# jedward225/MARL-HideAndSeek

Measured on AMD Instinct MI355X. Metric: world-steps/sec (agent-steps/sec derived) at 16K worlds, 1/2/4/8 GPU, higher is better.
Workload: dtype f32; 1 GPU; 16000 worlds/GPU x 2646 steps, 2 hiders + 2 seekers, sim_flags=0, rand_seed=0, random move actions in [-5,4] each step (scripts/benchmark.py args); worlds_per_gpu=16000, total_worlds=16000, agents_per_world=4

## Files before the change

__graft_entry__.py:

```python
import os
import sys

ROOT = os.path.dirname(os.path.abspath(__file__))
PKG = os.path.join(ROOT, "marl-hideandseek_amd")
for p in (PKG, os.path.join(ROOT, "oracle")):
    if p not in sys.path:
        sys.path.insert(0, p)


def build():
    import build as hs_build
    lib = hs_build.build_lib()
    hs_build.build_headless()
    hs_build.build_smallcap()
    import hs_ref
    hs_ref.build()
    import subprocess
    syms = ("hs_create", "hs_destroy", "hs_init", "hs_step", "hs_step_begin", "hs_step_end", "hs_step_async",
            "hs_get_tensor", "hs_train_interface", "hs_get_device_status", "hs_render", "hs_xla_init", "hs_xla_step",
            "hs_xla_save_checkpoints", "hs_xla_load_checkpoints", "hs_pack_policy_inputs", "hs_pack_policy_inputs_async")
    subprocess.check_call([sys.executable, "-c",
                           "import ctypes, sys; L = ctypes.CDLL(sys.argv[1]); [getattr(L, s) for s in sys.argv[2:]]", lib, *syms])
    subprocess.check_call([sys.executable, "-c", "import sys; sys.path.insert(0, sys.argv[1]); import gpu_hideseek", PKG])
    return lib


def smoke():
    import torch
    import lockstep
    assert torch.cuda.is_available(), "smoke() needs a GPU"
    p = lockstep.Pair(32, seed=7, render=(32, 32))
    p.drive(8, "bench", seed=0, every=8, walls=False,
            names=("self_data", "box_data", "lidar", "reward", "visible_boxes_mask"))
    p.sim.render()
    p.check_views(32, 32, "smoke")
    print("smoke OK: 8 steps x 32 worlds and their 128 agent views bit-exact vs oracle")


if __name__ == "__main__":
    if len(sys.argv) > 1 and sys.argv[1] == "smoke":
        smoke()
    else:
        print(build())
```

marl-hideandseek_amd/build.py:

```python
import os
import shutil
import subprocess
import sys

HERE = os.path.dirname(os.path.abspath(__file__))
CSRC = os.path.join(HERE, "csrc")
LIB = os.path.join(HERE, "lib", "libhideseek.so")

HIPCC_FLAGS = ["--offload-arch=gfx950", "-O3", "-fno-slp-vectorize", "-Wno-pass-failed", "-std=c++17", "-fPIC", "-shared", "-ffp-contract=off",
               "-fno-fast-math", "-Wno-unused-value"]


def sources():
    return sorted(os.path.join(CSRC, f) for f in os.listdir(CSRC) if f.endswith((".hip", ".h"))) + [
        os.path.join(os.path.dirname(HERE), "include", "hideseek.h")]


def up_to_date(lib=LIB):
    if not os.path.exists(lib):
        return False
    t = os.path.getmtime(lib)
    return all(os.path.getmtime(s) <= t for s in sources())


def build_lib(force=False, verbose=False, out=LIB, defines=()):
    if not force and up_to_date(out):
        return out
    hipcc = shutil.which("hipcc") or "/opt/rocm/bin/hipcc"
    if not os.path.exists(hipcc):
        raise RuntimeError("hipcc not found: cannot build libhideseek.so (there is no CPU fallback)")
    os.makedirs(os.path.dirname(out), exist_ok=True)
    cmd = [hipcc] + HIPCC_FLAGS + ["-D" + d for d in defines] + (
        ["-Rpass-analysis=kernel-resource-usage"] if verbose else []) + ["-o", out, os.path.join(CSRC, "hideseek.hip")]
    subprocess.check_call(cmd, cwd=CSRC)
    return out


SMALLCAP_LIB = os.path.join(HERE, "lib", "libhideseek_smallcap.so")


def build_smallcap(force=False):
    return build_lib(force=force, out=SMALLCAP_LIB, defines=("HS_MAX_DD_CAND=1", "HS_MAX_S_CAND=1"))


TIMING_LIB = os.path.join(HERE, "lib", "libhideseek_timing.so")


def build_timing(force=False):
    return build_lib(force=force, out=TIMING_LIB, defines=("HS_PHASE_TIMING",))


def build_headless():
    out = os.path.join(HERE, "lib", "headless")
    src = os.path.join(HERE, "tools", "headless.cpp")
    if os.path.exists(out) and os.path.getmtime(out) >= max(os.path.getmtime(src), os.path.getmtime(LIB)):
        return out
    subprocess.check_call(["g++", "-O2", "-std=c++17", "-I", os.path.join(os.path.dirname(HERE), "include"), src,
                           "-L", os.path.join(HERE, "lib"), "-lhideseek", "-Wl,-rpath,$ORIGIN", "-o", out])
    return out


if __name__ == "__main__":
    print(build_lib(force="--force" in sys.argv, verbose="-v" in sys.argv))
    print(build_headless())
    print(build_smallcap(force="--force" in sys.argv))
    if "--timing" in sys.argv:
        print(build_timing(force="--force" in sys.argv))
```

marl-hideandseek_amd/csrc/hs_dev.h:

```cpp
#pragma once
#include <hip/hip_runtime.h>
#include <stdint.h>

#define HSD __device__ __forceinline__

__device__ __forceinline__ int hs_lane() { int x = threadIdx.x; asm volatile("" : "+v"(x)); return x; }

namespace hs {

constexpr int kMaxBoxes = 9;
constexpr int kMaxRamps = 2;
constexpr int kMaxAgents = 6;
constexpr int kBoxSlot0 = 0;
constexpr int kRampSlot0 = 9;
constexpr int kAgentSlot0 = 11;
constexpr int kNumDSlots = 17;
constexpr int kMaxWalls = 36;
constexpr int kMaxPlanes = 3;
constexpr int kNumPrepSteps = 96;
constexpr int kEpisodeLen = 240;
constexpr int kNumSubsteps = 4;
constexpr float kSubstepH = (1.f / 30.f) / 4.f;
constexpr float kInvSubstepH = 120.f;
constexpr float kGravityZ = -9.8f;
constexpr float kMaxDepenVel = 3.f;
#ifndef HS_MAX_DD_CAND
#define HS_MAX_DD_CAND 16
#endif
#ifndef HS_MAX_S_CAND
#define HS_MAX_S_CAND 24
#endif
constexpr int kMaxDDCand = HS_MAX_DD_CAND;
constexpr int kGrabWords = 15;
constexpr int kMaxSCand = HS_MAX_S_CAND;
constexpr float kCosFovHalf = 0.382683426f;
constexpr float kPi = 3.14159265358979323846f;

enum : int { OBJ_SPHERE = 0, OBJ_PLANE = 1, OBJ_CUBE = 2, OBJ_WALL = 3, OBJ_HIDER = 4, OBJ_SEEKER = 5,
             OBJ_RAMP = 6, OBJ_BOX = 7, OBJ_NONE = -1 };
enum : int { OWNER_NONE = 0, OWNER_SEEKER = 1, OWNER_HIDER = 2, OWNER_UNOWNABLE = 3 };
enum : int { RESP_DYNAMIC = 0, RESP_KINEMATIC = 1, RESP_STATIC = 2 };
enum : int { AGENT_SEEKER = 0, AGENT_HIDER = 1 };
enum : uint32_t { FLAG_USE_FIXED_WORLD = 1, FLAG_IGNORE_EPISODE_LENGTH = 2, FLAG_RANDOM_FLIP_TEAMS = 4,
                  FLAG_ZERO_AGENT_VELOCITY = 8, FLAG_EXT_SKIP_OBSERVATIONS = 1u << 16, FLAG_EXT_RENDER = 1u << 17 };

HSD int meta_pack(int obj, int resp, int owner) { return (obj + 1) | (resp << 8) | (owner << 16); }
HSD int meta_obj(int m) { return (m & 0xff) - 1; }
HSD int meta_resp(int m) { return (m >> 8) & 0xff; }
HSD int meta_owner(int m) { return (m >> 16) & 0xff; }

struct V3 { float x, y, z; };
struct Q { float w, x, y, z; };

HSD V3 v3(float x, float y, float z) { return V3{x, y, z}; }
HSD V3 operator+(V3 a, V3 b) { return {a.x + b.x, a.y + b.y, a.z + b.z}; }
HSD V3 operator-(V3 a, V3 b) { return {a.x - b.x, a.y - b.y, a.z - b.z}; }
HSD V3 operator-(V3 a) { return {-a.x, -a.y, -a.z}; }
HSD V3 operator*(V3 a, float s) { return {a.x * s, a.y * s, a.z * s}; }
HSD V3 mulc(V3 a, V3 b) { return {a.x * b.x, a.y * b.y, a.z * b.z}; }
HSD float hs_fma(float a, float b, float c) { return __builtin_fmaf(a, b, c); }
HSD float dot(V3 a, V3 b) { return hs_fma(a.z, b.z, hs_fma(a.y, b.y, a.x * b.x)); }
HSD V3 cross(V3 a, V3 b) { return {hs_fma(a.y, b.z, -(a.z * b.y)), hs_fma(a.z, b.x, -(a.x * b.z)), hs_fma(a.x, b.y, -(a.y * b.x))}; }
HSD V3 madd(V3 a, V3 b, float s) { return {hs_fma(b.x, s, a.x), hs_fma(b.y, s, a.y), hs_fma(b.z, s, a.z)}; }
HSD V3 nmadd(V3 a, V3 b, float s) { return {hs_fma(-b.x, s, a.x), hs_fma(-b.y, s, a.y), hs_fma(-b.z, s, a.z)}; }
HSD float dot_add(V3 a, V3 b, float c) { return hs_fma(a.z, b.z, hs_fma(a.y, b.y, hs_fma(a.x, b.x, c))); }
HSD V3 cross_add(V3 a, V3 b, V3 c) {
    return {hs_fma(a.y, b.z, hs_fma(-a.z, b.y, c.x)), hs_fma(a.z, b.x, hs_fma(-a.x, b.z, c.y)), hs_fma(a.x, b.y, hs_fma(-a.y, b.x, c.z))};
}
HSD float len2(V3 a) { return dot(a, a); }
HSD float len(V3 a) { return sqrtf(dot(a, a)); }
HSD V3 normalize(V3 a) { float inv = 1.f / len(a); return a * inv; }
HSD V3 vsel(bool c, V3 a, V3 b) { return {c ? a.x : b.x, c ? a.y : b.y, c ? a.z : b.z}; }

HSD Q qmul(Q a, Q b) {
    return {hs_fma(-a.z, b.z, hs_fma(-a.y, b.y, hs_fma(-a.x, b.x, a.w * b.w))),
            hs_fma(-a.z, b.y, hs_fma(a.y, b.z, hs_fma(a.x, b.w, a.w * b.x))),
            hs_fma(a.z, b.x, hs_fma(a.y, b.w, hs_fma(-a.x, b.z, a.w * b.y))),
            hs_fma(a.z, b.w, hs_fma(-a.y, b.x, hs_fma(a.x, b.y, a.w * b.z)))};
}
HSD Q qinv(Q q) { return {q.w, -q.x, -q.y, -q.z}; }
HSD Q qnormalize(Q q) {
    float n2 = hs_fma(q.z, q.z, hs_fma(q.y, q.y, hs_fma(q.x, q.x, q.w * q.w)));
    float inv = 1.f / sqrtf(n2);
    return {q.w * inv, q.x * inv, q.y * inv, q.z * inv};
}
HSD V3 qrot(Q q, V3 v) {
    V3 p = {q.x, q.y, q.z};
    float s = q.w;
    float d2 = 2.f * dot(p, v);
    float s2 = 2.f * s;
    float k = hs_fma(s2, s, -1.f);
    V3 c = cross(p, v);
    return {hs_fma(s2, c.x, hs_fma(d2, p.x, k * v.x)), hs_fma(s2, c.y, hs_fma(d2, p.y, k * v.y)), hs_fma(s2, c.z, hs_fma(d2, p.z, k * v.z))};
}

HSD void hs_sincosf(float x, float *s_out, float *c_out) {
    const float two_over_pi = 0.63661977236758134308f;
    const float pio2_hi = 1.5707962512969970703125f;
    const float pio2_lo = 7.54978995489188216e-8f;
    float kf = x * two_over_pi;
    int k = (int)(kf + (kf >= 0.f ? 0.5f : -0.5f));
    float fk = (float)k;
    float r = (x - fk * pio2_hi) - fk * pio2_lo;
    float z = r * r;
    float sp = ((-1.9515295891e-4f * z + 8.3321608736e-3f) * z - 1.6666654611e-1f) * z * r + r;
    float cp = ((2.443315711809948e-5f * z - 1.388731625493765e-3f) * z + 4.166664568298827e-2f) * z * z
               - 0.5f * z + 1.f;
    int q = k & 3;
    float s = (q == 0) ? sp : (q == 1) ? cp : (q == 2) ? -sp : -cp;
    float c = (q == 0) ? cp : (q == 1) ? -sp : (q == 2) ? -cp : sp;
    *s_out = s; *c_out = c;
}
HSD float hs_atanf(float xin) {
    float sign = xin < 0.f ? -1.f : 1.f;
    float x = fabsf(xin);
    float y;
    const bool big = x > 2.414213562373095f, mid = x > 0.4142135623730950f;
    y = big ? 1.5707963267948966f : (mid ? 0.7853981633974483f : 0.f);
    if (mid) { const float num = big ? -1.f : x - 1.f, den = big ? x : x + 1.f; x = num / den; }
    float z = x * x;
    y = y + ((((8.05374449538e-2f * z - 1.38776856032e-1f) * z + 1.99777106478e-1f) * z - 3.33329491539e-1f) * z * x + x);
    return sign * y;
}
HSD float hs_atan2f(float y, float x) {
    if (x == 0.f) {
        if (y > 0.f) return 0.5f * kPi;
        if (y < 0.f) return -0.5f * kPi;
        return 0.f;
    }
    float a = hs_atanf(y / x);
    if (x < 0.f) { a = (y >= 0.f) ? a + kPi : a - kPi; }
    return a;
}
HSD float hs_asinf(float xin) {
    float sign = xin < 0.f ? -1.f : 1.f;
    float a = fabsf(xin);
    float z, x;
    bool flag = a > 0.5f;
    if (flag) { z = 0.5f * (1.f - a); x = sqrtf(z); }
    else { x = a; z = x * x; }
    float p = ((((4.2163199048e-2f * z + 2.4181311049e-2f) * z + 4.5470025998e-2f) * z + 7.4953002686e-2f) * z
               + 1.6666752422e-1f) * z * x + x;
    if (flag) { p = p + p; p = 1.5707963267948966f - p; }
    return sign * p;
}
HSD Q quat_angle_axis_z(float angle) {
    float s, c;
    hs_sincosf(angle * 0.5f, &s, &c);
    return {c, 0.f, 0.f, s};
}

struct M3 { V3 c0, c1, c2; };
HSD M3 m3_from_quat(Q q) {
    float y2 = q.y * q.y, z2 = q.z * q.z;
    float xy = q.x * q.y, xz = q.x * q.z, yz = q.y * q.z;
    M3 m;
    m.c0 = {hs_fma(-2.f, hs_fma(q.y, q.y, z2), 1.f), 2.f * hs_fma(q.w, q.z, xy), 2.f * hs_fma(-q.w, q.y, xz)};
    m.c1 = {2.f * hs_fma(-q.w, q.z, xy), hs_fma(-2.f, hs_fma(q.x, q.x, z2), 1.f), 2.f * hs_fma(q.w, q.x, yz)};
    m.c2 = {2.f * hs_fma(q.w, q.y, xz), 2.f * hs_fma(-q.w, q.x, yz), hs_fma(-2.f, hs_fma(q.x, q.x, y2), 1.f)};
    return m;
}

HSD V3 quat_to_euler(Q q) {
    float sinr = 2.f * (q.w * q.x + q.y * q.z);
    float cosr = 1.f - 2.f * (q.x * q.x + q.y * q.y);
    float roll = hs_atan2f(sinr, cosr);
    float sinp = 2.f * (q.w * q.y - q.z * q.x);
    float pitch = fabsf(sinp) >= 1.f ? copysignf(kPi / 2.f, sinp) : hs_asinf(sinp);
    float siny = 2.f * (q.w * q.z + q.x * q.y);
    float cosy = 1.f - 2.f * (q.y * q.y + q.z * q.z);
    float yaw = hs_atan2f(siny, cosy);
    return {roll, pitch, yaw};
}

struct RandKey { uint32_t a, b; };
HSD uint32_t rotl32(uint32_t x, int r) { return (x << r) | (x >> (32 - r)); }
HSD RandKey threefry2x32(RandKey key, uint32_t c0, uint32_t c1) {
    const uint32_t ks0 = key.a, ks1 = key.b, ks2 = 0x1BD11BDAu ^ key.a ^ key.b;
    uint32_t x0 = c0 + ks0, x1 = c1 + ks1;
#define HS_TF_R(r) { x0 += x1; x1 = rotl32(x1, r); x1 ^= x0; }
    HS_TF_R(13) HS_TF_R(15) HS_TF_R(26) HS_TF_R(6)
    x0 += ks1; x1 += ks2 + 1u;
    HS_TF_R(17) HS_TF_R(29) HS_TF_R(16) HS_TF_R(24)
    x0 += ks2; x1 += ks0 + 2u;
    HS_TF_R(13) HS_TF_R(15) HS_TF_R(26) HS_TF_R(6)
    x0 += ks0; x1 += ks1 + 3u;
    HS_TF_R(17) HS_TF_R(29) HS_TF_R(16) HS_TF_R(24)
// ... 43 lines not shown
```

marl-hideandseek_amd/csrc/hs_k_physics.h:

```cpp
#pragma once
#include "hs_state.h"
#include "hs_rays.h"
#include "hs_collide.h"
#include "hs_solver.h"
#include "hs_k_reset.h"

namespace hs {

constexpr int kPhysThreads = 64;
constexpr int kWorldLanes = kPhysThreads / kTile;
constexpr int kLdsWalls = 32;
static_assert(kMaxSCand <= 32 && kMaxDDCand <= 16, "accepted-manifold masks are one word per world");
constexpr int kAllDD = kNumDSlots * (kNumDSlots - 1) / 2;
constexpr int kAllSC = kNumDSlots * (kMaxWalls + kMaxPlanes - 1);
constexpr int kSpInfoWords = kNumDSlots + 1;

struct alignas(16) OctRes {
    static constexpr int kClip = kClipLanes;
    static constexpr int kClipWords = clip_words(kClip);
    static constexpr int kSatPairs = kClip < hs::kSatPairs ? kClip : hs::kSatPairs;
    static constexpr int kMaxItems = kTile * (kMaxDDCand + kMaxSCand);
    static constexpr int kSlots = kClip < 31 ? kClip : 31;
    static constexpr int kVelOffsetWords = 2 * 8 * 3 * 32;
    float pos[3][kNumDSlots][kTile];
// ... 36 lines not shown
};
static_assert(sizeof(OctRes) <= 20 * 1024, "8 waves of 8 worlds share the CU's 160 KiB of LDS");
static_assert(offsetof(OctRes, u.sat.items) >= offsetof(OctRes, u.det.wall), "items must not overlap the AABBs");
static_assert(sizeof(ManDD) / 4 * OctRes::kSlots <= OctRes::kVelOffsetWords, "manifold slots lie below the velocities");
static_assert(2 * 3 * kNumDSlots * 8 <= OctRes::kVelOffsetWords, "the hull AABBs lie below the velocities");

constexpr int kLocGlobal = 31;
HSD int pair_a(int p) { return p & 31; }
HSD int pair_b(int p) { return (p >> 5) & 63; }
HSD int pair_loc(int p) { return (p >> 11) & 31; }
HSD int pair_pack(int a, int b) { return a | (b << 5) | (kLocGlobal << 11); }
static_assert(kNumDSlots <= 32 && kMaxWalls + kMaxPlanes <= 64, "pair encoding");
static_assert(sizeof(ManDD) % 16 == 0 && sizeof(ManS) % 16 == 0, "manifold records move 16 bytes at a time");
constexpr int kManWords = sizeof(ManDD) / 4;
template <typename M> HSD void man_lds_load(const float *clip, int slot, M &m) {
    m = *reinterpret_cast<const M *>(clip + slot * kManWords);
}
template <typename M> HSD void man_lds_set_lam(float *clip, int slot, int j, float v) {
    static_assert(offsetof(M, lam) == sizeof(M) - 16, "lam is the record's tail");
    clip[slot * kManWords + (sizeof(M) / 4 - 4 + j)] = v;
}

template <int C> HSD V3 rld3(const float (&a)[C][kNumDSlots][kTile], int slot, int g) { return {a[0][slot][g], a[1][slot][g], a[2][slot][g]}; }
HSD Q rld4(const float (&a)[4][kNumDSlots][kTile], int slot, int g) { return {a[0][slot][g], a[1][slot][g], a[2][slot][g], a[3][slot][g]}; }
HSD void rst3(float (&a)[3][kNumDSlots][kTile], int slot, int g, V3 v) { a[0][slot][g] = v.x; a[1][slot][g] = v.y; a[2][slot][g] = v.z; }
HSD void rst4(float (&a)[4][kNumDSlots][kTile], int slot, int g, Q q) { a[0][slot][g] = q.w; a[1][slot][g] = q.x; a[2][slot][g] = q.y; a[3][slot][g] = q.z; }

HSD void rbody_load(const OctRes &R, int g, int slot, BodyS &b) {
    b.pos = rld3(R.pos, slot, g); b.rot = rld4(R.rot, slot, g);
    b.ppos = rld3(R.ppos, slot, g); b.prot = rld4(R.prot, slot, g);
    b.lin = rld3(R.u.vel.lin, slot, g); b.ang = rld3(R.u.vel.ang, slot, g);
    const int m = R.meta[slot][g];
    const bool dyn = m != 0 && meta_resp(m) == RESP_DYNAMIC;
    b.invM = dyn ? obj_inv_mass(meta_obj(m)) : 0.f;
    b.invI = dyn ? obj_inv_inertia(meta_obj(m)) : V3{0.f, 0.f, 0.f};
    body_refresh_inertia(b);
}
HSD void rbody_store_pose(OctRes &R, int g, int slot, const BodyS &b) { rst3(R.pos, slot, g, b.pos); rst4(R.rot, slot, g, b.rot); }
HSD void rbody_store_vel(OctRes &R, int g, int slot, const BodyS &b) { rst3(R.u.vel.lin, slot, g, b.lin); rst3(R.u.vel.ang, slot, g, b.ang); }
HSD void derive_velocity(BodyS &b) {
    const float h = kSubstepH;
    b.lin = (b.pos - b.ppos) * (1.f / h);
    Q dq = qmul(b.rot, qinv(b.prot));
    V3 wv = V3{dq.x, dq.y, dq.z} * (2.f / h);
    b.ang = dq.w >= 0.f ? wv : -wv;
}

HSD void wave_sync() { asm volatile("s_waitcnt lgkmcnt(0)" ::: "memory"); }
HSD void mem_sync() { asm volatile("s_waitcnt vmcnt(0) lgkmcnt(0)" ::: "memory"); }

template <int D> HSD int dpp_row_shr(int x) { return __builtin_amdgcn_update_dpp(0, x, 0x110 + D, 0xF, 0xF, true); }
HSD int scan8_incl(int x, int l) {
    int y;
    y = dpp_row_shr<1>(x); if (l >= 1) x += y;
    y = dpp_row_shr<2>(x); if (l >= 2) x += y;
    y = dpp_row_shr<4>(x); if (l >= 4) x += y;
    return x;
}
HSD int sum8_all(int x) {
    x += __builtin_amdgcn_update_dpp(0, x, 0xB1, 0xF, 0xF, false);
    x += __builtin_amdgcn_update_dpp(0, x, 0x4E, 0xF, 0xF, false);
    x += __builtin_amdgcn_update_dpp(0, x, 0x141, 0xF, 0xF, false);
    return x;
}
HSD int scan64_incl(int x) {
    x += dpp_row_shr<1>(x); x += dpp_row_shr<2>(x); x += dpp_row_shr<4>(x); x += dpp_row_shr<8>(x);
    x += __builtin_amdgcn_update_dpp(0, x, 0x142, 0xA, 0xF, false);
    x += __builtin_amdgcn_update_dpp(0, x, 0x143, 0xC, 0xF, false);
    return x;
}

struct ResGeom {
    const OctRes &R; const SimState &S; int g; int w;
    HSD int g_meta(int i) const { return R.meta[i][g]; }
    HSD V3 g_pos(int i) const { return rld3(R.pos, i, g); }
    HSD Q g_rot(int i) const { return rld4(R.rot, i, g); }
    HSD int g_num_walls() const { return R.numWalls[g]; }
    HSD float g_wall(int k, int c) const { return S.walls(c * kMaxWalls + k, w); }
    HSD int g_num_planes() const { return R.numPlanes[g]; }
    HSD float g_plane(int p, int c) const { return S.planes(c * kMaxPlanes + p, w); }
};

constexpr float kGroundOff = 0.f;
struct BodyReg {
    int np, vidx;
    float lam[4];
};

template <typename E, int ROWS>
HSD void copy_in(E *dst, const Col<E, ROWS> &col, int p0) {
    static_assert(sizeof(E) == 4, "16-byte pieces");
    const float4 *src = reinterpret_cast<const float4 *>(col.octet(p0 >> 3));
    float4 *d = reinterpret_cast<float4 *>(dst);
    for (int i = hs_lane(); i < ROWS * 2; i += 64) d[i] = src[(i / 2) * 2 + i % 2];
}
template <typename E, int ROWS>
HSD void copy_out(const Col<E, ROWS> &col, int p0, const E *src) {
    static_assert(sizeof(E) == 4, "16-byte pieces");
    float4 *dst = reinterpret_cast<float4 *>(col.octet(p0 >> 3));
    const float4 *s = reinterpret_cast<const float4 *>(src);
    for (int i = hs_lane(); i < ROWS * 2; i += 64) dst[(i / 2) * 2 + i % 2] = s[i];
}
HSD void copy_out_vel(const Col<float, 3 * kNumDSlots> &col, int p0, const float *src, const OctRes &R) {
    float *dst = col.octet(p0 >> 3);
    for (int i = hs_lane(); i < 3 * kNumDSlots * kTile; i += 64) {
        const int row = i / kTile, g = i % kTile, slot = row % kNumDSlots;
        const int m = R.meta[slot][g];
        if (m != 0 && meta_resp(m) == RESP_DYNAMIC) dst[row * kTile + g] = src[i];
    }
}

HSD void integrate_body(OctRes &R, BodyReg &b, int slot, int g, int meta, const float *aforce) {
    const int obj = meta_obj(meta);
    const bool dyn = meta_resp(meta) == RESP_DYNAMIC;
    V3 force = {0.f, 0.f, 0.f}; float torque = 0.f;
    if (dyn && slot >= kAgentSlot0) {
        const float *f = aforce + (slot - kAgentSlot0) * kTile + g;
        force = {f[0 * kMaxAgents * kTile], f[1 * kMaxAgents * kTile], f[2 * kMaxAgents * kTile]};
        torque = f[3 * kMaxAgents * kTile];
    }
    V3 pos = rld3(R.pos, slot, g); Q rot = rld4(R.rot, slot, g);
    rst3(R.ppos, slot, g, pos); rst4(R.prot, slot, g, rot);
    if (dyn) {
        V3 lin = rld3(R.u.vel.lin, slot, g), ang = rld3(R.u.vel.ang, slot, g);
        const float h = kSubstepH;
        const float invM = obj_inv_mass(obj);
        const V3 invI = obj_inv_inertia(obj);
        lin = madd(lin, madd(V3{0.f, 0.f, kGravityZ}, force, invM), h);
        pos = madd(pos, lin, h);
        Q qi = qinv(rot);
        V3 wloc = qrot(qi, ang), tl = qrot(qi, V3{0.f, 0.f, torque});
        const V3 I = obj_inertia(obj);
        V3 Iw = mulc(I, wloc);
        wloc = madd(wloc, mulc(invI, tl - cross(wloc, Iw)), h);
        ang = qrot(rot, wloc);
        rot = quat_add_rotation(rot, ang * h);
        rst3(R.pos, slot, g, pos); rst4(R.rot, slot, g, rot);
        rst3(R.u.vel.lin, slot, g, lin); rst3(R.u.vel.ang, slot, g, ang);
    }
    V3 lo, hi;
    const HullRef hb = hull_ref_body(obj, pos, rot);
    hull_aabb(hb, &lo, &hi);
    rst3(R.u.det.lo, slot, g, lo); rst3(R.u.det.hi, slot, g, hi);
    b.np = 0; b.vidx = 0;
#pragma unroll
    for (int j = 0; j < 4; ++j) b.lam[j] = 0.f;
    if (dyn && R.numPlanes[g] >= 1) {
        const V3 pn = {R.plane0[0][g], R.plane0[1][g], R.plane0[2][g]};
        b.np = ground_manifold(hb, pn, R.plane0[3][g], &b.vidx);
    }
}

struct ItemCounts { int nbox, nwedge; bool anySpill; };
template <int JB>
HSD ItemCounts phase_detect(const SimState &S, OctRes &R, int NS) {
    constexpr int G = kWorldLanes;
    const int L = hs_lane(), g = L / G, l = L % G;
    {
        constexpr int PR = kTile / 4;
        static_assert(kLdsWalls * PR <= 64, "one piece per lane per component");
        const float *src = S.walls.octet(S.wbeg >> 3);
        float4 v[4];
        const bool on = L < kLdsWalls * PR;
        const int row = L / PR, part = L % PR;
#pragma unroll
        for (int c = 0; c < 4; ++c) if (on) v[c] = *(const float4 *)(src + (c * kMaxWalls + row) * kTile + 4 * part);
#pragma unroll
        for (int c = 0; c < 4; ++c) if (on) *(float4 *)(&R.u.det.wall[c][row][4 * part]) = v[c];
    }
    if (l == 0) { R.scAcc[g] = 0u; R.ddAcc[g] = 0u; }
    wave_sync();
    const int nwl = R.numWalls[g], npl = R.numPlanes[g];
    int tot_items = 0;
    unsigned dd_mask[JB] = {}; unsigned long long s_mask[JB] = {};
    int bdd[JB] = {}, bsc[JB] = {}, add[JB] = {}, asc[JB] = {};
    bool have[JB], dynamic[JB]; V3 lo[JB], hi[JB];
#pragma unroll
    for (int jb = 0; jb < JB; ++jb) {
        const int slot = l + jb * G;
        const int meta = slot < NS ? R.meta[slot][g] : 0;
        have[jb] = meta != 0;
        dynamic[jb] = have[jb] && meta_resp(meta) == RESP_DYNAMIC;
        lo[jb] = {0.f, 0.f, 0.f}; hi[jb] = {0.f, 0.f, 0.f};
        if (have[jb]) { lo[jb] = rld3(R.u.det.lo, slot, g); hi[jb] = rld3(R.u.det.hi, slot, g); }
    }
#pragma unroll 4
    for (int j = 1; j < NS; ++j) {
        const int mj = R.meta[j][g];
        const bool dynj = meta_resp(mj) == RESP_DYNAMIC;
        const V3 loj = rld3(R.u.det.lo, j, g), hij = rld3(R.u.det.hi, j, g);
#pragma unroll
        for (int jb = 0; jb < JB; ++jb) {
            const bool hit = (mj != 0) & have[jb] & (l + jb * G < j) & (dynamic[jb] | dynj) &
                (lo[jb].x <= hij.x) & (loj.x <= hi[jb].x) & (lo[jb].y <= hij.y) & (loj.y <= hi[jb].y) &
                (lo[jb].z <= hij.z) & (loj.z <= hi[jb].z);
            dd_mask[jb] |= hit ? 1u << j : 0u;
        }
    }
    bool zin[JB];
#pragma unroll
    for (int jb = 0; jb < JB; ++jb) zin[jb] = dynamic[jb] & (lo[jb].z <= 2.5f) & (0.f <= hi[jb].z);
    auto wall_test = [&](int k, float cx, float cy, float hx, float hy) {
        const float wx0 = cx - hx, wx1 = cx + hx, wy0 = cy - hy, wy1 = cy + hy;
#pragma unroll
        for (int jb = 0; jb < JB; ++jb) {
            const bool hit = zin[jb] & (lo[jb].x <= wx1) & (wx0 <= hi[jb].x) & (lo[jb].y <= wy1) & (wy0 <= hi[jb].y);
            s_mask[jb] |= hit ? 1ull << k : 0ull;
        }
    };
    const int nwLds = nwl < kLdsWalls ? nwl : kLdsWalls;
#pragma unroll 4
    for (int k = 0; k < nwLds; ++k) wall_test(k, R.u.det.wall[0][k][g], R.u.det.wall[1][k][g], R.u.det.wall[2][k][g], R.u.det.wall[3][k][g]);
    for (int k = kLdsWalls; k < nwl; ++k) {
        const int w = S.wbeg + g;
        wall_test(k, S.walls(0 * kMaxWalls + k, w), S.walls(1 * kMaxWalls + k, w), S.walls(2 * kMaxWalls + k, w), S.walls(3 * kMaxWalls + k, w));
    }
    int tot_dd = 0, tot_sc = 0;
#pragma unroll
    for (int jb = 0; jb < JB; ++jb) {
        if (dynamic[jb]) for (int p = 1; p < npl; ++p) s_mask[jb] |= 1ull << (kMaxWalls + p);
        const int cdd = __popc(dd_mask[jb]), csc = __popcll(s_mask[jb]);
        const int in_dd = scan8_incl(cdd, l), in_sc = scan8_incl(csc, l);
        bdd[jb] = tot_dd + in_dd - cdd; bsc[jb] = tot_sc + in_sc - csc;
        tot_dd += sum8_all(cdd); tot_sc += sum8_all(csc);
        add[jb] = cdd ? max(0, min(cdd, kMaxDDCand - bdd[jb])) : 0;
        asc[jb] = csc ? max(0, min(csc, kMaxSCand - bsc[jb])) : 0;
        tot_items += add[jb] + asc[jb];
        if (add[jb] != cdd) atomicAdd(&S.status[0], cdd - add[jb]);
        if (asc[jb] != csc) atomicAdd(&S.status[1], csc - asc[jb]);
    }
    const bool spillDD = tot_dd > kMaxDDCand, spillSC = tot_sc > kMaxSCand;
    const bool anySpill = __ballot(spillDD || spillSC) != 0ull;
    unsigned short *const spPair = S.spPair + (size_t)(S.wbeg + g) * (kAllDD + kAllSC);
    int *const spInfo = S.spInfo + (size_t)(S.wbeg + g) * kSpInfoWords;
    int n_wedge = 0;
#pragma unroll
    for (int jb = 0; jb < JB; ++jb) {
        const int slot = l + jb * G;
        const bool ramp = slot >= kRampSlot0 && slot < kRampSlot0 + kMaxRamps;
        if (ramp) n_wedge += add[jb] + asc[jb];
        else { unsigned mm = dd_mask[jb]; for (int i = 0; mm && i < add[jb]; ++i) { const int j = __ffs(mm) - 1; mm &= mm - 1; n_wedge += (j >= kRampSlot0 && j < kRampSlot0 + kMaxRamps) ? 1 : 0; } }
    }
    const int n_box = tot_items - n_wedge;
    const int inc_box = scan64_incl(n_box), inc_wedge = scan64_incl(n_wedge);
    ItemCounts ic;
    ic.anySpill = anySpill;
    ic.nbox = __builtin_amdgcn_readlane(inc_box, 63); ic.nwedge = __builtin_amdgcn_readlane(inc_wedge, 63);
    const int wedge0 = (ic.nbox + 31) / 32 * 32;
    int ibox = inc_box - n_box, iwedge = wedge0 + inc_wedge - n_wedge;
    wave_sync();
#pragma unroll
    for (int jb = 0; jb < JB; ++jb) {
        const int slot = l + jb * G;
        const bool ramp = slot >= kRampSlot0 && slot < kRampSlot0 + kMaxRamps;
        unsigned mm = dd_mask[jb]; int i = 0;
        while (mm && i < add[jb]) {
            const int j = __ffs(mm) - 1; mm &= mm - 1;
            R.ddPair[bdd[jb] + i][g] = (unsigned short)pair_pack(slot, j);
            const unsigned short item = (unsigned short)((g << 6) | (bdd[jb] + i));
            if (ramp || (j >= kRampSlot0 && j < kRampSlot0 + kMaxRamps)) R.u.sat.items[iwedge++] = item; else R.u.sat.items[ibox++] = item;
            ++i;
        }
        while (mm) {
            const int j = __ffs(mm) - 1; mm &= mm - 1;
            spPair[bdd[jb] + i] = (unsigned short)pair_pack(slot, j);
            ++i;
        }
        unsigned long long sm = (s_mask[jb] >> kMaxWalls) | (s_mask[jb] << (64 - kMaxWalls) >> (64 - kMaxWalls) << kMaxPlanes); i = 0;
        while (sm && i < asc[jb]) {
            const int bit = __ffsll((long long)sm) - 1; sm &= sm - 1;
            const int k = bit < kMaxPlanes ? kMaxWalls + bit : bit - kMaxPlanes;
            R.scPair[bsc[jb] + i][g] = (unsigned short)pair_pack(slot, k);
            const unsigned short item = (unsigned short)((g << 6) | 32 | (bsc[jb] + i));
            if (ramp) R.u.sat.items[iwedge++] = item; else R.u.sat.items[ibox++] = item;
            ++i;
        }
        const int nspill = sm ? __popcll(sm) : 0;
        while (sm) {
            const int bit = __ffsll((long long)sm) - 1; sm &= sm - 1;
            const int k = bit < kMaxPlanes ? kMaxWalls + bit : bit - kMaxPlanes;
            spPair[kAllDD + bsc[jb] + i] = (unsigned short)pair_pack(slot, k);
            ++i;
        }
        if (spillSC && slot < kNumDSlots) spInfo[1 + slot] = nspill ? ((bsc[jb] + asc[jb]) | (nspill << 16)) : 0;
        if (slot < NS) R.scInfo[slot][g] = (unsigned short)(asc[jb] > 0 ? (bsc[jb] | (asc[jb] << 8)) : 0);
    }
    if (l == 0) {
        R.spill[g] = (unsigned char)((spillDD ? 1 : 0) | (spillSC ? 2 : 0));
        if (spillDD || spillSC) spInfo[0] = tot_dd | (tot_sc << 16);
        R.ndd[g] = (unsigned char)min(tot_dd, kMaxDDCand); R.nsc[g] = (unsigned char)min(tot_sc, kMaxSCand);
        if (R.wid[g] >= 0 && tot_dd + tot_sc > 0) S.loadAcc[R.wid[g]] += tot_dd + tot_sc;
    }
    wave_sync();
    return ic;
}

template <bool POS, int UNROLL, typename SetLam>
HSD void static_manifold(BodyS &me, const ManS &m, SetLam set_lam) {
    BodyS none;
    body_refresh_inertia(me);
    const V3 n = ld3(m.n);
    const int np = m.np;
    const float mu = POS ? m.muS : m.muD;
#pragma unroll UNROLL
    for (int j = 0; j < 4; ++j)
        if (j < np) {
            const float lamj = m.lam[j];
            if (POS) set_lam(j, lamj + solve_point_position<false>(me, none, n, ld3(m.rA[j]), V3{0.f, 0.f, 0.f}, m.offB[j], mu));
            else solve_point_velocity<false>(me, none, n, ld3(m.rA[j]), V3{0.f, 0.f, 0.f}, lamj, mu);
        }
}

#define HS_COLD __device__ __forceinline__
struct SpillCtx {
    const float *walls, *planes;
    ManDD *wsDD; ManS *wsSC; unsigned short *spPair; int *spInfo;
    int wbeg;
};
HSD SpillCtx spill_ctx(const SimState &S) { return {S.walls.p, S.planes.p, (ManDD *)S.wsDD, (ManS *)S.wsSC, S.spPair, S.spInfo, S.wbeg}; }

HS_COLD void spill_sat(SpillCtx c, OctRes *Rp) {
    OctRes &R = *Rp;
    const int lane = hs_lane() & 63;
    const bool hi = (lane & 1) != 0;
    const Col<float, 4 * kMaxWalls> walls = {const_cast<float *>(c.walls)};
    const Col<float, 4 * kMaxPlanes> planes = {const_cast<float *>(c.planes)};
#pragma unroll 1
    for (int g = 0; g < kTile; ++g) {
        const int fl = __builtin_amdgcn_readfirstlane((int)R.spill[g]);
        if (fl == 0) continue;
        const int w = c.wbeg + g;
        const int tot = __builtin_amdgcn_readfirstlane(c.spInfo[(size_t)w * kSpInfoWords]);
#pragma unroll 1
        for (int kind = 0; kind < 2; ++kind) {
            if ((fl & (1 << kind)) == 0) continue;
            const bool isdd = kind == 0;
            const int n = isdd ? tot & 0xffff : tot >> 16;
#pragma unroll 1
            for (int base = isdd ? kMaxDDCand : kMaxSCand; base < n; base += OctRes::kSatPairs) {
                const int kk = base + (lane >> 1);
                if (kk < n && (lane >> 1) < OctRes::kSatPairs) {
                    const int pair = c.spPair[(size_t)w * (kAllDD + kAllSC) + (isdd ? 0 : kAllDD) + kk];
                    const int a = pair_a(pair), bsel = pair_b(pair);
                    const int oa = meta_obj(R.meta[a][g]);
                    const V3 pa = rld3(R.pos, a, g);
                    const Q qa = rld4(R.rot, a, g);
                    ManDD *const md = c.wsDD + (size_t)w * kAllDD + kk;
                    ManS *const ms = c.wsSC + (size_t)w * kAllSC + kk;
                    RawManifold raw;
                    raw.np = 0;
                    bool plane = false;
                    if (!isdd && bsel >= kMaxWalls) {
                        const int p = bsel - kMaxWalls;
                        const V3 pn = {planes(0 * kMaxPlanes + p, w), planes(1 * kMaxPlanes + p, w), planes(2 * kMaxPlanes + p, w)};
                        plane = true;
                        if (!hi && !collide_hull_plane(hull_ref_body(oa, pa, qa), pn, planes(3 * kMaxPlanes + p, w), raw)) raw.np = 0;
                    } else {
                        const HullSrc ha = hull_src_body(oa, pa, qa);
                        const HullSrc hb = isdd ? hull_src_body(meta_obj(R.meta[bsel][g]), rld3(R.pos, bsel, g), rld4(R.rot, bsel, g))
                                                : hull_src_wall(walls(0 * kMaxWalls + bsel, w), walls(1 * kMaxWalls + bsel, w),
                                                                walls(2 * kMaxWalls + bsel, w), walls(3 * kMaxWalls + bsel, w));
                        const AxisResult res = sat_axes(ha, hb, hi);
                        const ClipBuf cb = {R.u.sat.clip, lane >> 1, OctRes::kClip};
                        if (!hi && res.code != 0 && !sat_contact(ha, hb, res, cb, raw)) raw.np = 0;
                    }
                    if (!hi) {
                        const int ob = isdd ? meta_obj(R.meta[bsel][g]) : plane ? OBJ_PLANE : OBJ_WALL;
                        const float muS = 0.5f * (obj_mu_s(oa) + obj_mu_s(ob)), muD = 0.5f * (obj_mu_d(oa) + obj_mu_d(ob));
// ... 733 lines not shown
            const bool hidden = hider_reward == 1.f;
            const bool sf = cnt_seekers_first(counts) != 0;
            const int win = hidden ? (sf ? 1 : 0) : (sf ? 0 : 1);
            if (win == 0) s0 += 1; else s1 += 1;
        }
        if (step == kEpisodeLen - 1) {
            if (s0 > s1) { res[0] = 1.f; res[1] = 0.f; }
            else if (s0 < s1) { res[0] = 0.f; res[1] = 1.f; }
            else { res[0] = 0.5f; res[1] = 0.5f; }
        }
        S.runningScores(0, p) = s0; S.runningScores(1, p) = s1;
        S.hiderTeamReward[w] = hider_reward;
    }
}

template <int ROUNDS, int LASTR, bool POS>
HSD void static_passes(const SimState &S, OctRes &R, BodyReg (&br)[ROUNDS], int nbodies, int nLast, int nMerged) {
    const int L = hs_lane();
#pragma unroll
    for (int r = 0; r < LASTR; ++r) {
        const bool valid = r * 64 + L < nbodies; const int t_ = valid ? R.bodies[r * 64 + L] : 0;
        const int slot = t_ >> 3, g = t_ & 7; const int meta = valid ? R.meta[slot][g] : 0;
        if (valid) { if (POS) ground_pos(R, br[r], slot, g, meta); else ground_vel(R, br[r], slot, g, meta); }
    }
    wave_sync();
    {
        const bool valid = LASTR * 64 + L < nbodies; const int t_ = valid ? R.bodies[LASTR * 64 + L] : 0;
        const int slot = t_ >> 3, g = t_ & 7; const int meta = valid ? R.meta[slot][g] : 0;
        last_round<POS>(S, R, br[LASTR], valid, slot, g, meta, nLast, nMerged);
    }
    wave_sync();
}

#ifdef HS_PHASE_TIMING
#define HS_TICK_PARAMS , long long &tk, long long (&acc)[10]
#define HS_TICK_ARGS , tk, acc
#define HS_TICK(i) { const long long now_ = wall_clock64(); acc[i] += now_ - tk; tk = now_; }
#else
#define HS_TICK_PARAMS
#define HS_TICK_ARGS
#define HS_TICK(i)
#endif
#define HS_BODY(r) const bool valid = (r) * 64 + L < nbodies; const int t_ = valid ? R.bodies[(r) * 64 + L] : 0; \
                   const int slot = t_ >> 3, g = t_ & 7; const int meta = valid ? R.meta[slot][g] : 0;
template <int ROUNDS>
HSD void substep_rest(const SimState &S, OctRes &R, BodyReg (&br)[ROUNDS], int nbodies, int NS, ItemCounts ic, bool integrateNext,
                      const float *aforce HS_TICK_PARAMS) {
    const int L = hs_lane();
    const bool manGlobal = phase_sat(S, R, ic);
    HS_TICK(3)
    phase_dd<true>(S, R, ic.anySpill);
    HS_TICK(4)
    constexpr int kShortLastR = ROUNDS - 2;
    const bool shortLast = ROUNDS == 3 && nbodies <= 64 * (ROUNDS - 1);
    const int lastRound = shortLast ? kShortLastR : ROUNDS - 1;
    const WallLists wl = list_wall_bodies<ROUNDS>(R, nbodies, lastRound);
    const int nLast = max(nbodies - 64 * lastRound, 0);
    const int nMerged = min(wl.nEarly, 64 - nLast);
    if (shortLast) static_passes<ROUNDS, kShortLastR, true>(S, R, br, nbodies, nLast, nMerged);
    else static_passes<ROUNDS, ROUNDS - 1, true>(S, R, br, nbodies, nLast, nMerged);
    if (wl.nwb > nMerged) { wall_round<true>(S, R, nMerged, wl.nwb); wave_sync(); }
    if (__builtin_expect(ic.anySpill, 0)) { spill_static<true>(spill_ctx(S), &R, NS); wave_sync(); }
#pragma unroll
    for (int r = 0; r < ROUNDS; ++r) { HS_BODY(r) if (valid) derive_body_velocity(R, slot, g, meta); }
    if (manGlobal) mem_sync(); else wave_sync();
    HS_TICK(5)
    phase_dd<false>(S, R, ic.anySpill);
    HS_TICK(6)
    if (shortLast) static_passes<ROUNDS, kShortLastR, false>(S, R, br, nbodies, nLast, nMerged);
    else static_passes<ROUNDS, ROUNDS - 1, false>(S, R, br, nbodies, nLast, nMerged);
    if (wl.nwb > nMerged) { wall_round<false>(S, R, nMerged, wl.nwb); wave_sync(); }
    if (__builtin_expect(ic.anySpill, 0)) { spill_static<false>(spill_ctx(S), &R, NS); wave_sync(); }
    if (integrateNext) {
#pragma unroll
        for (int r = 0; r < ROUNDS; ++r) { HS_BODY(r) if (valid) integrate_body(R, br[r], slot, g, meta, aforce); }
        wave_sync();
    }
    HS_TICK(7)
}

template <int ROUNDS>
HSD void physics_step(SimState &S, OctRes &R, GenScratch *gen) {
    const int L = hs_lane(), o = blockIdx.x;
    S.wbeg = o * kTile;
    const int p0 = S.wbeg;
    const int NS = kAgentSlot0 + S.A;
    const int noct = gridDim.x;
    const long long tStart = wall_clock64();
    {
        const int sidx = S.stepIdx, prevIdx = sidx == 0 ? 2 : sidx - 1, nextIdx = sidx == 2 ? 0 : sidx + 1;
        if (o == 0 && L == 0) S.tickSum[nextIdx] = 0ull;
        const float mean = (float)S.tickSum[prevIdx] / (float)noct, mine = (float)S.octTicks[o];
        const bool known = mean > 0.f;
        if (known && mine > 1.10f * mean) __builtin_amdgcn_s_setprio(3);
        else if (known && mine > 0.98f * mean) __builtin_amdgcn_s_setprio(2);
        else if (known && mine > 0.88f * mean) __builtin_amdgcn_s_setprio(1);
        else if (known) __builtin_amdgcn_s_setprio(0);
        else __builtin_amdgcn_s_setprio(2);
    }
#ifdef HS_PHASE_TIMING
    long long tk = wall_clock64(); long long acc[10] = {0, 0, 0, 0, 0, 0, 0, 0, 0, 0};
#endif
    copy_in(&R.pos[0][0][0], S.bpos, p0); copy_in(&R.rot[0][0][0], S.brot, p0);
    copy_in(&R.u.vel.lin[0][0][0], S.blin, p0); copy_in(&R.u.vel.ang[0][0][0], S.bang, p0);
    copy_in(&R.meta[0][0], S.bmeta, p0);
    if (L < kTile) {
        const int w = S.worldOfSlot[S.wbeg + L];
        R.wid[L] = w;
        R.numWalls[L] = w >= 0 ? (unsigned char)S.numWalls[w] : 0;
        R.numPlanes[L] = w >= 0 ? (unsigned char)S.numPlanes[w] : 0;
        R.seen[L] = 0; R.ndd[L] = 0; R.nsc[L] = 0;
        R.wallSeen[L] = w >= 0 ? (unsigned)S.wallHist[w] : 0u;
    }
    if (L < 4 * kTile) (&R.plane0[0][0])[L] = S.planes((L / kTile) * kMaxPlanes, S.wbeg + (L % kTile));
    wave_sync();
    HS_TICK(9)
    phase_pre(S, R);
    HS_TICK(0)
    int nbodies;
    {
        int base = 0;
#pragma unroll
        for (int pass = 0; pass < 2; ++pass) {
#pragma unroll
            for (int c = 0; c < ROUNDS; ++c) {
                const int t = c * 64 + L;
                const int ord = t / kTile, g = t % kTile;
                const int slot = ord < S.A ? kAgentSlot0 + ord : ord - S.A;
                const bool hist = ord < NS && ((R.wallSeen[g] >> slot) & 1u) != 0u;
                const bool on = ord < NS && R.meta[slot][g] != 0 && hist == (pass == 0);
                const unsigned long long m = __ballot(on);
                if (on) R.bodies[base + __popcll(m & ((1ull << L) - 1ull))] = (unsigned char)(slot << 3 | g);
                base += __popcll(m);
            }
        }
        nbodies = base;
    }
    wave_sync();
    if (L < kTile) R.wallSeen[L] = 0u;
    wave_sync();
    BodyReg br[ROUNDS];
    const float *const aforce = S.aforce.octet(p0 >> 3);
#pragma unroll
    for (int r = 0; r < ROUNDS; ++r) {
        BodyReg &b = br[r];
        b.np = 0; b.vidx = 0;
#pragma unroll
        for (int j = 0; j < 4; ++j) b.lam[j] = 0.f;
        HS_BODY(r)
        if (valid) integrate_body(R, b, slot, g, meta, aforce);
    }
    wave_sync();
    HS_TICK(1)
#pragma unroll 1
    for (int sub = 0; sub < kNumSubsteps; ++sub) {
        const ItemCounts ic = phase_detect<ROUNDS>(S, R, NS);
        HS_TICK(2)
        substep_rest<ROUNDS>(S, R, br, nbodies, NS, ic, sub + 1 < kNumSubsteps, aforce HS_TICK_ARGS);
    }
#undef HS_BODY
    phase_post(S, R);
    wave_sync();
    copy_out(S.bpos, p0, &R.pos[0][0][0]); copy_out(S.brot, p0, &R.rot[0][0][0]);
    copy_out_vel(S.blin, p0, &R.u.vel.lin[0][0][0], R); copy_out_vel(S.bang, p0, &R.u.vel.ang[0][0][0], R);
    copy_out(S.bmeta, p0, &R.meta[0][0]);
    mem_sync();
    HS_TICK(8)
    {
        const int myWorld = L < kTile ? R.wid[L] : -1;
        const int mySeen = L < kTile ? (int)R.wallSeen[L] : 0;
        wave_sync();
        if (myWorld >= 0) {
            S.wallHist[myWorld] = mySeen;
            reset_world(S, myWorld, gen[L]);
        }
    }
    if (L == 0) {
        const int dt = (int)(wall_clock64() - tStart);
        S.octTicks[o] = dt;
        atomicAdd(&S.tickSum[S.stepIdx], (unsigned long long)dt);
    }
#ifdef HS_PHASE_TIMING
    if (L == 0) for (int i = 0; i < 10; ++i) S.phaseTicks[(size_t)o * 10 + i] += acc[i];
#endif
#undef HS_TICK
}

template <int ROUNDS>
__global__ void __launch_bounds__(kPhysThreads, 2) k_physics(SimState S) {
    __shared__ union PhysLds { OctRes R; GenScratch gen[kTile]; } lds;
    static_assert(sizeof(PhysLds) <= 20 * 1024, "8 waves of 8 worlds share the CU's 160 KiB of LDS");
    physics_step<ROUNDS>(S, lds.R, lds.gen);
}

}
```

Baseline: 32.43 million world-steps/s.

## Cache inflated broadphase candidate sets across substeps with fp16-packed bounds

Adds a conservative broadphase prefilter: on the first substep, or whenever any body leaves its cached bounds, each body's AABB is inflated by a margin plus three times its displacement, packed to fp16 with outward rounding, and used to build per-world candidate masks for body-body and wall pairs. On later substeps the exact tests run only over the cached candidate bits instead of scanning all bodies and walls, and the wall LDS staging is skipped. This removes repeated O(N) broadphase scans per substep but costs extra registers, per-world divergent bit-iteration loops, and global wall loads in the sparse path.

```diff
diff --git a/__graft_entry__.py b/__graft_entry__.py
--- a/__graft_entry__.py
+++ b/__graft_entry__.py
@@ -13,6 +13,7 @@
     lib = hs_build.build_lib()
     hs_build.build_headless()
     hs_build.build_smallcap()
+    hs_build.build_zeromargin()
     import hs_ref
     hs_ref.build()
     import subprocess
diff --git a/marl-hideandseek_amd/build.py b/marl-hideandseek_amd/build.py
--- a/marl-hideandseek_amd/build.py
+++ b/marl-hideandseek_amd/build.py
@@ -43,6 +43,13 @@
     return build_lib(force=force, out=SMALLCAP_LIB, defines=("HS_MAX_DD_CAND=1", "HS_MAX_S_CAND=1"))
 
 
+ZEROMARGIN_LIB = os.path.join(HERE, "lib", "libhideseek_zeromargin.so")
+
+
+def build_zeromargin(force=False):
+    return build_lib(force=force, out=ZEROMARGIN_LIB, defines=("HS_PREFILTER_MARGIN_MM=0",))
+
+
 TIMING_LIB = os.path.join(HERE, "lib", "libhideseek_timing.so")
 
 
@@ -64,5 +71,6 @@
     print(build_lib(force="--force" in sys.argv, verbose="-v" in sys.argv))
     print(build_headless())
     print(build_smallcap(force="--force" in sys.argv))
+    print(build_zeromargin(force="--force" in sys.argv))
     if "--timing" in sys.argv:
         print(build_timing(force="--force" in sys.argv))
diff --git a/marl-hideandseek_amd/csrc/hs_dev.h b/marl-hideandseek_amd/csrc/hs_dev.h
--- a/marl-hideandseek_amd/csrc/hs_dev.h
+++ b/marl-hideandseek_amd/csrc/hs_dev.h
@@ -33,6 +33,10 @@
 constexpr int kMaxDDCand = HS_MAX_DD_CAND;
 constexpr int kGrabWords = 15;
 constexpr int kMaxSCand = HS_MAX_S_CAND;
+#ifndef HS_PREFILTER_MARGIN_MM
+#define HS_PREFILTER_MARGIN_MM 50
+#endif
+constexpr float kPrefilterMargin = HS_PREFILTER_MARGIN_MM * 0.001f;
 constexpr float kCosFovHalf = 0.382683426f;
 constexpr float kPi = 3.14159265358979323846f;
 
diff --git a/marl-hideandseek_amd/csrc/hs_k_physics.h b/marl-hideandseek_amd/csrc/hs_k_physics.h
--- a/marl-hideandseek_amd/csrc/hs_k_physics.h
+++ b/marl-hideandseek_amd/csrc/hs_k_physics.h
@@ -212,29 +212,40 @@
 }
 
 struct ItemCounts { int nbox, nwedge; bool anySpill; };
+typedef __fp16 half2_t __attribute__((ext_vector_type(2)));
+struct WideBox { V3 lo, hi; };
+struct WidePacked { half2_t x, y, z; };
+HSD half2_t wide_pack1(float lo, float hi, float d) {
+    constexpr float m = kPrefilterMargin, far = 60000.f;
+    const float t = (m > 0.f ? 3.f : 0.f) * d;
+    const unsigned p = __builtin_bit_cast(unsigned, __builtin_amdgcn_cvt_pkrtz(fmaxf(lo + fminf(t, 0.f) - m, -far), fminf(hi + fmaxf(t, 0.f) + m, far)));
+    return __builtin_bit_cast(half2_t, p + ((p >> 15) & 1u) + ((~p >> 15) & 0x10000u));
+}
+HSD WidePacked wide_pack(V3 lo, V3 hi, V3 d) { return {wide_pack1(lo.x, hi.x, d.x), wide_pack1(lo.y, hi.y, d.y), wide_pack1(lo.z, hi.z, d.z)}; }
+HSD WideBox wide_unpack(WidePacked p) { return {{(float)p.x.x, (float)p.y.x, (float)p.z.x}, {(float)p.x.y, (float)p.y.y, (float)p.z.y}}; }
+template <int JB> struct WideSet {
+    WidePacked box[JB];
+    unsigned dd; unsigned long long s;
+};
+template <int JB> HSD WideSet<JB> wide_none() {
+    WideSet<JB> ws;
+    const half2_t none = {(__fp16)__builtin_inff(), (__fp16)__builtin_inff()};
+#pragma unroll
+    for (int jb = 0; jb < JB; ++jb) ws.box[jb] = {none, none, none};
+    ws.dd = 0u; ws.s = 0ull;
+    return ws;
+}
 template <int JB>
-HSD ItemCounts phase_detect(const SimState &S, OctRes &R, int NS) {
+HSD ItemCounts phase_detect(const SimState &S, OctRes &R, int NS, WideSet<JB> &ws) {
     constexpr int G = kWorldLanes;
     const int L = hs_lane(), g = L / G, l = L % G;
-    {
-        constexpr int PR = kTile / 4;
-        static_assert(kLdsWalls * PR <= 64, "one piece per lane per component");
-        const float *src = S.walls.octet(S.wbeg >> 3);
-        float4 v[4];
-        const bool on = L < kLdsWalls * PR;
-        const int row = L / PR, part = L % PR;
-#pragma unroll
-        for (int c = 0; c < 4; ++c) if (on) v[c] = *(const float4 *)(src + (c * kMaxWalls + row) * kTile + 4 * part);
-#pragma unroll
-        for (int c = 0; c < 4; ++c) if (on) *(float4 *)(&R.u.det.wall[c][row][4 * part]) = v[c];
-    }
     if (l == 0) { R.scAcc[g] = 0u; R.ddAcc[g] = 0u; }
-    wave_sync();
     const int nwl = R.numWalls[g], npl = R.numPlanes[g];
     int tot_items = 0;
     unsigned dd_mask[JB] = {}; unsigned long long s_mask[JB] = {};
     int bdd[JB] = {}, bsc[JB] = {}, add[JB] = {}, asc[JB] = {};
     bool have[JB], dynamic[JB]; V3 lo[JB], hi[JB];
+    bool outside = false;
 #pragma unroll
     for (int jb = 0; jb < JB; ++jb) {
         const int slot = l + jb * G;
@@ -243,37 +254,92 @@
         dynamic[jb] = have[jb] && meta_resp(meta) == RESP_DYNAMIC;
         lo[jb] = {0.f, 0.f, 0.f}; hi[jb] = {0.f, 0.f, 0.f};
         if (have[jb]) { lo[jb] = rld3(R.u.det.lo, slot, g); hi[jb] = rld3(R.u.det.hi, slot, g); }
-    }
+        const WideBox in = wide_unpack(ws.box[jb]);
+        outside |= have[jb] & !((lo[jb].x >= in.lo.x) & (lo[jb].y >= in.lo.y) & (lo[jb].z >= in.lo.z) &
+                                (hi[jb].x <= in.hi.x) & (hi[jb].y <= in.hi.y) & (hi[jb].z <= in.hi.z));
+    }
+    auto dd_hit = [&](int jb, int j, int mj, V3 alo, V3 ahi, V3 blo, V3 bhi) {
+        return (mj != 0) & have[jb] & (l + jb * G < j) & (dynamic[jb] | (meta_resp(mj) == RESP_DYNAMIC)) &
+            (alo.x <= bhi.x) & (blo.x <= ahi.x) & (alo.y <= bhi.y) & (blo.y <= ahi.y) & (alo.z <= bhi.z) & (blo.z <= ahi.z);
+    };
+    auto wall_hit = [&](int jb, V3 alo, V3 ahi, float cx, float cy, float hx, float hy) {
+        const float wx0 = cx - hx, wx1 = cx + hx, wy0 = cy - hy, wy1 = cy + hy;
+        return dynamic[jb] & (alo.z <= 2.5f) & (0.f <= ahi.z) & (alo.x <= wx1) & (wx0 <= ahi.x) & (alo.y <= wy1) & (wy0 <= ahi.y);
+    };
+    const bool full = __ballot(outside) != 0ull;
+#ifdef HS_PF_COUNT
+    if (L == 0) { atomicAdd(&S.status[1], 1); if (full) atomicAdd(&S.status[0], 1); }
+#endif
+    if (full) {
+        {
+            constexpr int PR = kTile / 4;
+            static_assert(kLdsWalls * PR <= 64, "one piece per lane per component");
+            const float *src = S.walls.octet(S.wbeg >> 3);
+            float4 v[4];
+            const bool on = L < kLdsWalls * PR;
+            const int row = L / PR, part = L % PR;
+#pragma unroll
+            for (int c = 0; c < 4; ++c) if (on) v[c] = *(const float4 *)(src + (c * kMaxWalls + row) * kTile + 4 * part);
+#pragma unroll
+            for (int c = 0; c < 4; ++c) if (on) *(float4 *)(&R.u.det.wall[c][row][4 * part]) = v[c];
+        }
+        wave_sync();
+        WideBox wb[JB];
+        bool lost = false;
+#pragma unroll
+        for (int jb = 0; jb < JB; ++jb) {
+            const int slot = l + jb * G;
+            const V3 d = have[jb] ? rld3(R.pos, slot, g) - rld3(R.ppos, slot, g) : V3{0.f, 0.f, 0.f};
+            ws.box[jb] = wide_pack(lo[jb], hi[jb], d); wb[jb] = wide_unpack(ws.box[jb]);
+            lost |= have[jb] & !((lo[jb].x >= wb[jb].lo.x) & (lo[jb].y >= wb[jb].lo.y) & (lo[jb].z >= wb[jb].lo.z) &
+                                 (hi[jb].x <= wb[jb].hi.x) & (hi[jb].y <= wb[jb].hi.y) & (hi[jb].z <= wb[jb].hi.z));
+        }
+        ws.dd = 0u; ws.s = 0ull;
 #pragma unroll 4
-    for (int j = 1; j < NS; ++j) {
-        const int mj = R.meta[j][g];
-        const bool dynj = meta_resp(mj) == RESP_DYNAMIC;
-        const V3 loj = rld3(R.u.det.lo, j, g), hij = rld3(R.u.det.hi, j, g);
-#pragma unroll
-        for (int jb = 0; jb < JB; ++jb) {
-            const bool hit = (mj != 0) & have[jb] & (l + jb * G < j) & (dynamic[jb] | dynj) &
-                (lo[jb].x <= hij.x) & (loj.x <= hi[jb].x) & (lo[jb].y <= hij.y) & (loj.y <= hi[jb].y) &
-                (lo[jb].z <= hij.z) & (loj.z <= hi[jb].z);
-            dd_mask[jb] |= hit ? 1u << j : 0u;
-        }
-    }
-    bool zin[JB];
-#pragma unroll
-    for (int jb = 0; jb < JB; ++jb) zin[jb] = dynamic[jb] & (lo[jb].z <= 2.5f) & (0.f <= hi[jb].z);
-    auto wall_test = [&](int k, float cx, float cy, float hx, float hy) {
-        const float wx0 = cx - hx, wx1 = cx + hx, wy0 = cy - hy, wy1 = cy + hy;
-#pragma unroll
-        for (int jb = 0; jb < JB; ++jb) {
-            const bool hit = zin[jb] & (lo[jb].x <= wx1) & (wx0 <= hi[jb].x) & (lo[jb].y <= wy1) & (wy0 <= hi[jb].y);
-            s_mask[jb] |= hit ? 1ull << k : 0ull;
-        }
-    };
-    const int nwLds = nwl < kLdsWalls ? nwl : kLdsWalls;
+        for (int j = 1; j < NS; ++j) {
+            const int mj = R.meta[j][g];
+            const WideBox wj = wide_unpack(wide_pack(rld3(R.u.det.lo, j, g), rld3(R.u.det.hi, j, g), rld3(R.pos, j, g) - rld3(R.ppos, j, g)));
+            bool hit = false;
+#pragma unroll
+            for (int jb = 0; jb < JB; ++jb) hit |= dd_hit(jb, j, mj, wb[jb].lo, wb[jb].hi, wj.lo, wj.hi);
+            ws.dd |= hit ? 1u << j : 0u;
+        }
+        auto wall_wide = [&](int k, float cx, float cy, float hx, float hy) {
+            bool hit = false;
+#pragma unroll
+            for (int jb = 0; jb < JB; ++jb) hit |= wall_hit(jb, wb[jb].lo, wb[jb].hi, cx, cy, hx, hy);
+            ws.s |= hit ? 1ull << k : 0ull;
+        };
+        const int nwLds = nwl < kLdsWalls ? nwl : kLdsWalls;
 #pragma unroll 4
-    for (int k = 0; k < nwLds; ++k) wall_test(k, R.u.det.wall[0][k][g], R.u.det.wall[1][k][g], R.u.det.wall[2][k][g], R.u.det.wall[3][k][g]);
-    for (int k = kLdsWalls; k < nwl; ++k) {
+        for (int k = 0; k < nwLds; ++k) wall_wide(k, R.u.det.wall[0][k][g], R.u.det.wall[1][k][g], R.u.det.wall[2][k][g], R.u.det.wall[3][k][g]);
+        for (int k = kLdsWalls; k < nwl; ++k) {
+            const int w = S.wbeg + g;
+            wall_wide(k, S.walls(0 * kMaxWalls + k, w), S.walls(1 * kMaxWalls + k, w), S.walls(2 * kMaxWalls + k, w), S.walls(3 * kMaxWalls + k, w));
+        }
+        if (__ballot(lost) != 0ull) { ws.dd = ~0u >> (32 - NS) & ~1u; ws.s = nwl ? ~0ull >> (64 - nwl) : 0ull; }
+    }
+    {
+        unsigned ud = ws.dd; unsigned long long us = ws.s;
         const int w = S.wbeg + g;
-        wall_test(k, S.walls(0 * kMaxWalls + k, w), S.walls(1 * kMaxWalls + k, w), S.walls(2 * kMaxWalls + k, w), S.walls(3 * kMaxWalls + k, w));
+        auto wall_load = [&](int k) { return float4{S.walls(0 * kMaxWalls + k, w), S.walls(1 * kMaxWalls + k, w), S.walls(2 * kMaxWalls + k, w), S.walls(3 * kMaxWalls + k, w)}; };
+        int k = us ? __ffsll((long long)us) - 1 : 0;
+        float4 wk = wall_load(k);
+        while (ud) {
+            const int j = __ffs(ud) - 1; ud &= ud - 1;
+            const int mj = R.meta[j][g];
+            const V3 loj = rld3(R.u.det.lo, j, g), hij = rld3(R.u.det.hi, j, g);
+#pragma unroll
+            for (int jb = 0; jb < JB; ++jb) dd_mask[jb] |= dd_hit(jb, j, mj, lo[jb], hi[jb], loj, hij) ? 1u << j : 0u;
+        }
+        while (us) {
+            const int kc = k; const float4 wc = wk;
+            us &= us - 1;
+            k = us ? __ffsll((long long)us) - 1 : 0;
+            wk = wall_load(k);
+#pragma unroll
+            for (int jb = 0; jb < JB; ++jb) s_mask[jb] |= wall_hit(jb, lo[jb], hi[jb], wc.x, wc.y, wc.z, wc.w) ? 1ull << kc : 0ull;
+        }
     }
     int tot_dd = 0, tot_sc = 0;
 #pragma unroll
@@ -1313,9 +1379,10 @@
     }
     wave_sync();
     HS_TICK(1)
+    WideSet<ROUNDS> wide = wide_none<ROUNDS>();
 #pragma unroll 1
     for (int sub = 0; sub < kNumSubsteps; ++sub) {
-        const ItemCounts ic = phase_detect<ROUNDS>(S, R, NS);
+        const ItemCounts ic = phase_detect<ROUNDS>(S, R, NS, wide);
         HS_TICK(2)
         substep_rest<ROUNDS>(S, R, br, nbodies, NS, ic, sub + 1 < kNumSubsteps, aforce HS_TICK_ARGS);
     }
```

Result: no change. 32.51 million world-steps/s, median of 3 (+0.2%).
